# dvnam1605/MAACO-path-planing

Hardware: NVIDIA B200
Metric: path evals/sec (MAACO ant tours, MPA/PSO/GA fitness) at 1/2/4/8 B200 vs CPU (higher is better)
Workload: dtype f64

## Files before the change

### maaco_path_planing_b200/csrc/mpp_maaco.cu

```cuda
#include <type_traits>
#include <cmath>
#include <cstdlib>
#include <thread>
#include <vector>

#include "mpp_common.cuh"

static inline double hdist(int r0, int c0, int r1, int c1) {
    long long dr = r0 - r1, dc = c0 - c1;
    return std::sqrt((double)(dr * dr + dc * dc));
}

extern "C" double mpp_maaco_q0(int K, int k, double q0_initial) {
    double k0 = 0.7 * (double)K, q0;
    if ((double)k < k0) {
        if (std::fabs((double)K - k0) < 1e-6) q0 = q0_initial;
        else q0 = ((double)(K - k) / (double)K) * q0_initial;
    } else {
        double q0_at_k0 = (((double)K - k0) / (double)K) * q0_initial;
        q0 = q0_at_k0 +
             (((double)k - k0) / ((double)K - k0 + 1e-9)) * (q0_initial * (1 - ((double)K - k0) / (double)K) / 2.0);
    }
    q0 = q0 > 0.01 ? q0 : 0.01;
    return q0 < 0.99 ? q0 : 0.99;
// ... 466 lines not shown
        const uint32_t need0 = __ballot_sync(0xffffffffu, active && ((unsigned)lrow - edge_lo > edge_span || (unsigned)lcol - edge_lo > edge_span));
        if (!__any_sync(0xffffffffu, active)) break;
        if ((step & gmask) == 0 || need0) {
            if ((step & gmask) == 0) {
                const int la = lane & (apw - 1);
                const mpp_u4 rb = mpp_philox(step + (uint32_t)(lane / apw), (uint32_t)(A.ant_offset + a0 + la), A.it,
                                             MPP_CLS_MAACO_TOUR, key0, key1);
                const double u0 = mpp_u53(rb.x, rb.y), u1 = mpp_u53(rb.z, rb.w);
                const bool greedy = u0 <= A.q0;
                uint32_t pack = greedy ? (1u << 24) : 0u;
#pragma unroll
                for (int n = 2; n <= 8; ++n) {
                    int k = (int)(u1 * (double)n);
                    k = k < n ? k : n - 1;
                    pack |= (uint32_t)k << (3 * (n - 1));
                }
                const uint32_t k2 = (pack >> 3) & 7u, k3 = (pack >> 6) & 7u;
                uint32_t pack2 = (greedy ? (1u << 16) : 0u) | (0u << 2) | (1u << 4) | (2u << 8);
                pack2 |= (k2 ? 1u : 0u) << 6;
                pack2 |= (k2 ? 2u : 0u) << 10;
                pack2 |= (k2 ? 2u : 1u) << 12;
                pack2 |= k3 << 14;
                __syncwarp();
                rngu[lane] = make_double2(u0, u1);
                rngp[lane] = pack;
                rngq[lane] = pack2;
                __syncwarp();
            }
            uint32_t need = need0;
            while (need) {
                const int src = __ffs(need) - 1;
                const int s_lrow = __shfl_sync(0xffffffffu, lrow, src), s_lcol = __shfl_sync(0xffffffffu, lcol, src);
                const int s_wr = __shfl_sync(0xffffffffu, wr, src), s_wc = __shfl_sync(0xffffffffu, wc, src);
                const int a_s = a0 + src;
                uint2 *const w_s = win_w + src * 64;
                int d_wr = 0, d_wc = 0;
                if ((unsigned)s_lrow - edge_lo > edge_span) {
                    const bool up = s_lrow < U;
                    d_wr = up ? -1 : 1;
                    const int t_out = up ? s_wr + 1 : s_wr, t_in = up ? s_wr - 1 : s_wr + 2;
                    const uint2 keep = w_s[up ? lane : lane + 32], out = w_s[up ? lane + 32 : lane];
                    tour_tile_store(V, a_s, t_out, s_wc, lane, out.x);
                    tour_tile_store(V, a_s, t_out, s_wc + 1, lane, out.y);
                    uint2 nw;
                    nw.x = tour_tile_load(V, a_s, t_in, s_wc, lane);
                    nw.y = tour_tile_load(V, a_s, t_in, s_wc + 1, lane);
                    w_s[up ? lane + 32 : lane] = keep;
                    w_s[up ? lane : lane + 32] = nw;
                } else {
                    const bool left = s_lcol < U;
                    d_wc = left ? -1 : 1;
                    const int t_out = left ? s_wc + 1 : s_wc, t_in = left ? s_wc - 1 : s_wc + 2;
                    const uint2 o0 = w_s[lane], o1 = w_s[lane + 32];
                    tour_tile_store(V, a_s, s_wr, t_out, lane, left ? o0.y : o0.x);
                    tour_tile_store(V, a_s, s_wr + 1, t_out, lane, left ? o1.y : o1.x);
                    const uint32_t x0 = tour_tile_load(V, a_s, s_wr, t_in, lane);
                    const uint32_t x1 = tour_tile_load(V, a_s, s_wr + 1, t_in, lane);
                    w_s[lane] = left ? make_uint2(x0, o0.x) : make_uint2(o0.y, x0);
                    w_s[lane + 32] = left ? make_uint2(x1, o1.x) : make_uint2(o1.y, x1);
                }
#ifdef MPP_TOUR_STATS
                if (lane == src) ++st_slides;
#endif
                if (lane == src) {
                    wr += d_wr; wc += d_wc;
                    lrow -= d_wr << 5; lcol -= d_wc << 5;
                    prow_s -= (uint32_t)(d_wr * 256);
                }
                __syncwarp();
                const bool again = (lane == src) && ((unsigned)lrow - edge_lo > edge_span || (unsigned)lcol - edge_lo > edge_span);
                need = (need & (need - 1)) | __ballot_sync(0xffffffffu, again);
            }
        }
        uint32_t slot = (step & gmask) * slot_bytes;
        for (int su = 0; su < U; ++su, slot += slot_bytes)
        if (active) {
            int m = -1, dcur = 0, dpr = 0, dcc = 0, dphi = 0;
            double dl = 0.0;
            if (!(fw2 & 1u)) {
                const uint32_t p2 = lds_u32(rngq_s + slot);
                const uint32_t A3 = (fw2 >> 1) & 7u;
                uint32_t pool;
#ifdef MPP_TOUR_STATS
                if (gap == 0) ++st_t1; else ++st_t2;
#endif
                if (gap == 0) {
                    pool = (p2 & 0x10000u) ? ((fw2 >> 25) & 7u) : A3;
                } else {
                    const uint2 ra = lds_u2(prow_s + k_dpr0), rb = lds_u2(prow_s + k_dpr1), rc = lds_u2(prow_s + k_dpr2);
                    const int c0 = lcol + k_dc0, c1 = lcol + k_dc1, c2 = lcol + k_dc2;
                    const uint32_t v0 = ((c0 & 32) ? ra.y : ra.x) >> (c0 & 31);
                    const uint32_t v1 = ((c1 & 32) ? rb.y : rb.x) >> (c1 & 31);
                    const uint32_t v2 = ((c2 & 32) ? rc.y : rc.x) >> (c2 & 31);
                    const uint32_t c3 = A3 & ~((v0 & 1u) | ((v1 & 1u) << 1) | ((v2 & 1u) << 2));
                    pool = (p2 & 0x10000u) ? ((fw2 >> (1u + 3u * c3)) & 7u) : c3;
                    if (c3 == 0u) pool = 0u;
                }
                if (pool != 0u) {
                    const uint32_t mem = (p2 >> (2u * pool)) & 3u;
                    const uint4 fv = lds_u4(sbase_k + T1_FAST_OFF + 16u * mem);
                    dl = lds_f64(sbase_k + T1_FLEN_OFF + 8u * mem);
                    dcur = (int)fv.x; dpr = (int)fv.y; dcc = (int)fv.z;
                    m = (int)(fv.w & 0xFFu);
                    dphi = (int)(fv.w >> 8);
                    const uint32_t m1 = 0u - (mem & 1u), m2 = 0u - (mem >> 1);
                    uint32_t t;
                    asm("lop3.b32 %0, %1, %2, %3, 0xD8;" : "=r"(t) : "r"(bq.x), "r"(bq.y), "r"(m1));
                    asm("lop3.b32 %0, %1, %2, %3, 0xD8;" : "=r"(fw2) : "r"(t), "r"(bq.z), "r"(m2));
                }
            }
#ifdef MPP_TOUR_STATS
            if (m < 0) { ++st_t3; if (!(fw2 & 1u)) { if (gap == 0) --st_t1; else --st_t2; } }
#endif
            if (m < 0) {
                const uint32_t ctx = (n_path >= 2) ? (uint32_t)(prev_m + 1) : 0u;
                const uint32_t fw = ldg32_nc_pinned(rank_fast + (size_t)cur * 9 + ctx);
                const uint2 rws = ldg64_pinned(rank_slow + (size_t)cur * 9 + ctx);
                uint2 nb = make_uint2(0u, 0u);
                if (fast_ok) nb = ldg64_pinned(nb8 + cur);
                const uint32_t pack = lds_u32(rngp_s + slot);
                const uint2 q0r = lds_u2(prow_s - 8u), q1r = lds_u2(prow_s), q2r = lds_u2(prow_s + 8u);
                const int rot = lcol - 1;
                const bool sw = rot & 32;
                const uint32_t t3 = __funnelshift_r(sw ? q0r.y : q0r.x, q0r.y, rot) & 7u;
                const uint32_t m3 = __funnelshift_r(sw ? q1r.y : q1r.x, q1r.y, rot) & 5u;
                const uint32_t b3 = __funnelshift_r(sw ? q2r.y : q2r.x, q2r.y, rot) & 7u;
                const uint32_t vis = t3 | ((m3 & 1u) << 3) | ((m3 & 4u) << 2) | (b3 << 5);
                const uint32_t valid = (fw >> 24) & ~vis;
                uint32_t cand = valid & P1;
                if (cand == 0u) {
                    cand = valid & orient_mask(tr - cur / C, tc - cur % C);
                    if (!cand) cand = valid;
                }
                if (cand == 0u) {
                    failed = true;
                    active = false;
                } else {
                    if ((cand & (cand - 1u)) == 0u) {
                        m = __ffs(cand) - 1;
                    } else if ((fw & 7u) != 0u) {
                        const double2 uu = rngu[(slot >> 2) + lane];
                        m = tour_select_slow(cand, cur / C, cur % C, C, n_path >= 2, prev_m, tau_m, E01_m, A.alpha, A.q0, uu.x, uu.y);
                    } else {
                        uint32_t pool = cand;
                        if (pack & (1u << 24)) {
                            const uint2 sp = lds_u2(sbase_k + T1_SPREAD_OFF + 8u * cand);
                            const uint32_t f0 = __byte_perm(sp.x, sp.y, rws.x & 0xFFFFu), f1 = __byte_perm(sp.x, sp.y, rws.x >> 16);
                            const uint32_t ff = f0 ? f0 : f1;
                            const int pos4 = ((__ffs(ff) - 1) >> 1) + (f0 ? 0 : 16);
                            const uint32_t best = (rws.x >> pos4) & 7u;
                            pool = cand & ~((1u << best) - 1u);
                        }
                        const int n = __popc(pool);
                        const int k = (pack >> (3 * n - 3)) & 7u;
                        m = (int)lds_u8(sbase_k + T1_KTH_OFF + pool * 8u + (uint32_t)k);
                    }
                    const uint4 mvv = lds_u4(sbase_k + T1_MOVE_OFF + 16u * (uint32_t)m);
                    dcur = (int)mvv.x; dpr = (int)mvv.y; dcc = (int)mvv.z; dphi = (int)mvv.w;
                    dl = lds_f64(sbase_k + T1_DLEN_OFF + 8u * (uint32_t)m);
                    if (fast_ok) {
                        const uint32_t by = (((m & 4) ? nb.y : nb.x) >> (8 * (m & 3))) & 0xFFu;
                        const uint32_t fl = lds_u32(sbase_k + T1_FLD_OFF + 4u * (by >> 4));
                        const uint32_t A3n = (by >> 1) & 7u;
                        const uint32_t Gn = A3n ? ((fl >> (3u * (A3n - 1u))) & 7u) : 0u;
                        fw2 = (by & 1u) | (A3n << 1) | (fl << 4) | (Gn << 25);
                    }
                }
            }
            if (active) {
                cur += dcur;
                if (fast_ok) bq = ldg128_pinned(bundle + cur);
                gap -= dphi;
                gap = gap > 0 ? gap : 0;
                prow_s += (uint32_t)dpr;
                lrow += dpr >> 3;
                lcol += dcc;
                asm volatile("red.shared.or.b32 [%0], %1;" ::"r"(prow_s + 4u * ((uint32_t)lcol >> 5)), "r"(1u << (lcol & 31)) : "memory");
                if (n_path <= k_max_cells) *mvp = (uint8_t)m;
                ++mvp;
                len += dl;
                if (m != prev_m) ++turns;
                prev_m = m;
                ++n_path;
                if (cur == k_target || n_path >= k_max_path) active = false;
#ifdef MPP_TOUR_STATS
                st_c1 = clock64();
#endif
            }
        }
    }
    for (int src = 0; src < apw && a0 + src < A.n_ants; ++src) {
        const int s_wr = __shfl_sync(0xffffffffu, wr, src), s_wc = __shfl_sync(0xffffffffu, wc, src);
        const uint2 o0 = win_w[src * 64 + lane], o1 = win_w[src * 64 + lane + 32];
        tour_tile_store(V, a0 + src, s_wr, s_wc, lane, o0.x);
        tour_tile_store(V, a0 + src, s_wr, s_wc + 1, lane, o0.y);
        tour_tile_store(V, a0 + src, s_wr + 1, s_wc, lane, o1.x);
        tour_tile_store(V, a0 + src, s_wr + 1, s_wc + 1, lane, o1.y);
    }
    if (lane < apw && a < A.n_ants) {
        const bool ok = !failed && cur == target;
        mpp_ant_result res;
        res.length = ok ? len : __longlong_as_double(0x7ff0000000000000ll);
        res.n_cells = ok ? n_path : 0;
        res.turns = ok ? (turns > 0 ? turns : 0) : -1;
        A.result[(size_t)map * A.result_stride + A.ant_offset + a] = res;
        if constexpr (P2P)
            for (int g = 0; g < PA.n_peers; ++g) PA.peer_result[g][A.ant_offset + a] = res;
        if (A.steps) atomicAdd(A.steps, (unsigned long long)(n_path - 1));
#ifdef MPP_TOUR_STATS
        int *st = (int *)(A.moves + ((size_t)map * A.n_ants + a + 1) * A.max_cells - 32);
        st[0] = st_t1; st[1] = st_t2; st[2] = st_t3; st[3] = st_slides; st[4] = (int)(st_c1 - st_c0); st[5] = n_path - 1;
        st[6] = ok ? 1 : 0;
#endif
    }
}

static int colony_check(const mpp_map_batch *maps, const mpp_colony *c, const char *who) {
    MPP_REQUIRE(maps && c, "%s: null argument", who);
    MPP_REQUIRE(c->tau && c->E01 && c->rank && c->slabs && c->touched && c->moves && c->result && c->deposit && c->okbits &&
                    c->state && c->best_cells && c->seeds, "%s: null colony buffer", who);
    MPP_REQUIRE(c->max_cells > 0 && c->tau_stride >= (long long)maps->rows * maps->cols, "%s: bad max_cells / tau_stride", who);
    for (int k = 0; k < maps->n_maps; ++k)
        MPP_REQUIRE(maps->meta_host[k].start >= 0 && maps->meta_host[k].target >= 0, "%s: map %d has no start/target", who, k);
    return MPP_OK;
}

static int tours_launch(const mpp_map_batch *maps, const mpp_colony *c, int iteration, double q0, double alpha,
                        int n_ants, int ant_offset, int n_ants_total, int ants_per_warp,
                        uint32_t *const *peer_slabs, uint32_t *const *peer_touched, mpp_ant_result *const *peer_result,
                        int n_peers, int rows_per_rank, void *stream) {
    int rc = colony_check(maps, c, "mpp_maaco_tours");
    if (rc) return rc;
    MPP_REQUIRE(n_ants > 0 && ant_offset >= 0 && ant_offset + n_ants <= n_ants_total, "mpp_maaco_tours: bad ant range");
    MPP_CUDA(cudaSetDevice(maps->device));
    const RankLayout L = rank_layout(maps->rows, maps->cols);
    const int TR = tiles_r(maps->rows);
    TourArgs A;
    A.meta = maps->meta_dev;
    A.rank = c->rank; A.rank_stride = L.total_words; A.rank_margin = L.margin; A.rank_fast_words = L.fast_words;
    A.rank_bundle_words = L.bundle_words; A.rank_nb8_words = L.nb8_words;
    A.R = maps->rows; A.C = maps->cols;
    A.tau = c->tau; A.tau_stride = (size_t)c->tau_stride; A.E01 = c->E01; A.E01_stride = (size_t)c->E01_stride;
    A.it = (uint32_t)iteration; A.q0 = q0; A.alpha = alpha;
    A.n_ants = n_ants; A.ant_offset = ant_offset;
    A.seeds = c->seeds;
    const size_t tw = (size_t)mpp_maaco_touched_words(TR, maps->cols, n_ants) / 2;
    A.slabs = c->slabs; A.slab_stride = (size_t)mpp_maaco_slab_words(TR, maps->cols, n_ants);
    A.touched = c->touched + (size_t)(iteration & 1) * tw * maps->n_maps; A.touched_stride = tw;
    A.moves = c->moves; A.max_cells = c->max_cells;
    A.result = c->result; A.result_stride = (size_t)n_ants_total;
    A.steps = c->steps; A.latch = c->latch;
    TourPeers PA;
    for (int g = 0; g < MPP_MAX_PEERS; ++g) {
        PA.peer_slabs[g] = g < n_peers ? peer_slabs[g] : nullptr;
        PA.peer_touched[g] = g < n_peers ? peer_touched[g] : nullptr;
        PA.peer_result[g] = g < n_peers ? peer_result[g] : nullptr;
    }
    PA.n_peers = n_peers; PA.rows_per_rank = rows_per_rank; PA.n_total = n_ants_total;
    int apw = 16;
    const char *e = getenv("MPP_TOUR_APW");
    if (e) apw = atoi(e);
    else if (ants_per_warp) apw = ants_per_warp;
    else {
        const long long total = (long long)n_ants * maps->n_maps;
        while (apw > 2 && (total + apw - 1) / apw < 12ll * maps->sm_count) apw >>= 1;
    }
    MPP_REQUIRE(apw == 1 || apw == 2 || apw == 4 || apw == 8 || apw == 16 || apw == 32,
                "ants per warp (MPP_TOUR_APW / ants_per_warp) must be a power of two <= 32");
    const int warps = (n_ants + apw - 1) / apw, wpb = MPP_TOUR1_THREADS / 32;
    const size_t smem = T1_WIN_OFF + (size_t)wpb * apw * 512;
    {
        static size_t smem_set[64] = {0};
        const int dv = maps->device & 63;
        if (smem > smem_set[dv]) {
            MPP_CUDA(cudaFuncSetAttribute(mpp_maaco_tour1_kernel<false>, cudaFuncAttributeMaxDynamicSharedMemorySize, (int)smem));
            MPP_CUDA(cudaFuncSetAttribute(mpp_maaco_tour1_kernel<true>, cudaFuncAttributeMaxDynamicSharedMemorySize, (int)smem));
            smem_set[dv] = smem;
        }
    }
    const dim3 grid((warps + wpb - 1) / wpb, maps->n_maps);
    if (n_peers > 0) mpp_maaco_tour1_kernel<true><<<grid, MPP_TOUR1_THREADS, smem, (cudaStream_t)stream>>>(A, apw, PA);
    else mpp_maaco_tour1_kernel<false><<<grid, MPP_TOUR1_THREADS, smem, (cudaStream_t)stream>>>(A, apw, TourNoPeers());
    MPP_CUDA(cudaGetLastError());
    return MPP_OK;
}

extern "C" int mpp_maaco_tours(const mpp_map_batch *maps, const mpp_colony *c, int iteration, double q0, double alpha,
                               int n_ants, int ant_offset, int n_ants_total, int ants_per_warp, void *stream) {
    return tours_launch(maps, c, iteration, q0, alpha, n_ants, ant_offset, n_ants_total, ants_per_warp, nullptr, nullptr,
                        nullptr, 0, 1, stream);
}

extern "C" int mpp_maaco_tours_p2p(const mpp_map_batch *maps, const mpp_colony *c, int iteration, double q0, double alpha,
                                   int n_ants, int ant_offset, int n_ants_total, int ants_per_warp,
                                   uint32_t *const *slabs_peers, uint32_t *const *touched_peers,
                                   mpp_ant_result *const *result_peers, int n_peers, int tile_rows_per_rank, void *stream) {
    MPP_REQUIRE(maps && maps->n_maps == 1, "mpp_maaco_tours_p2p: a sharded colony is one map");
    MPP_REQUIRE(slabs_peers && touched_peers && result_peers && n_peers > 0 && n_peers <= MPP_MAX_PEERS && tile_rows_per_rank > 0 &&
                    (long long)n_peers * tile_rows_per_rank >= tiles_r(maps->rows), "mpp_maaco_tours_p2p: bad peer arguments");
    return tours_launch(maps, c, iteration, q0, alpha, n_ants, ant_offset, n_ants_total, ants_per_warp, slabs_peers,
                        touched_peers, result_peers, n_peers, tile_rows_per_rank, stream);
}

__global__ void __launch_bounds__(128) mpp_maaco_rank_kernel(const uint8_t *__restrict__ svalid_all,
                                                             const double *__restrict__ tau_all, size_t tau_stride,
                                                             const double *__restrict__ E01_all, size_t E01_stride,
                                                             double alpha, int R, int C,
                                                             const MppMapMeta *__restrict__ meta, uint32_t *__restrict__ rank_all,
                                                             size_t rank_stride, size_t rank_margin, size_t rank_fast_words,
                                                             size_t rank_bundle_words, size_t rank_nb8_words,
                                                             const int32_t *__restrict__ latch) {
    const int cell = blockIdx.x * 128 + threadIdx.x;
    if (cell >= R * C) return;
    if (latch && *latch) return;
    const int map = blockIdx.y;
    const uint8_t *svalid = svalid_all + (size_t)map * R * C;
    const double *tau = tau_all + (size_t)map * tau_stride;
    const double *E01 = E01_all + (size_t)map * E01_stride;
    uint32_t *rank_fast = rank_all + (size_t)map * rank_stride + rank_margin;
    uint2 *rank_slow = (uint2 *)(rank_all + (size_t)map * rank_stride + rank_fast_words);
    uint32_t *bundle = rank_all + (size_t)map * rank_stride + rank_bundle_words;
    uint8_t *nb8 = (uint8_t *)(rank_all + (size_t)map * rank_stride + rank_nb8_words);
    const uint32_t P1 = meta[map].s1.P1;
    const uint32_t sv = svalid[cell];
    double a0[8], a1[8];
#pragma unroll
    for (int m = 0; m < 8; ++m) {
        a0[m] = a1[m] = -1.0;
        if ((sv >> m) & 1u) {
            const int j = cell + ((int)((0xA940u >> (2 * m)) & 3u) - 1) * C + ((int)((0x9224u >> (2 * m)) & 3u) - 1);
            const double tv = tau[j];
            const double ta = (alpha == 1.0) ? tv : pow_slow(tv, alpha);
            const double2 e = *(const double2 *)(E01 + 2 * (size_t)j);
            a0[m] = ta * e.x;
            a1[m] = ta * e.y;
        }
    }
    const bool p1_three = __popc(P1) == 3;
    const int s0 = __ffs(P1) - 1, s1 = __ffs(P1 & (P1 - 1)) - 1, s2 = 31 - __clz(P1);
    for (int ctx = 0; ctx < 9; ++ctx) {
        double a[8];
#pragma unroll
        for (int m = 0; m < 8; ++m) a[m] = (ctx > 0 && m != ctx - 1) ? a1[m] : a0[m];
        double cmx = 0.0;
#pragma unroll
        for (int m = 0; m < 8; ++m) cmx = fmax(cmx, a[m]);
        uint32_t word = 0xFFFFFFu, perm = 0u, fast = 7u, order = 0u;
        if (cmx < 1e-10) {
            word = 0u;
#pragma unroll
            for (int m = 0; m < 8; ++m) {
                int pos = 0;
#pragma unroll
                for (int q = 0; q < 8; ++q) pos += (a[q] > a[m]) || (a[q] == a[m] && q < m);
                word |= (uint32_t)pos << (3 * m);
                perm |= (uint32_t)m << (4 * pos);
            }
            fast = 0u;
            if (p1_three) {
                const uint32_t p0 = (word >> (3 * s0)) & 7u, p1 = (word >> (3 * s1)) & 7u, p2 = (word >> (3 * s2)) & 7u;
                order = (p0 < p1 ? 1u : 0u) | (p0 < p2 ? 2u : 0u) | (p1 < p2 ? 4u : 0u);
#pragma unroll
                for (uint32_t c = 1; c < 8; ++c) {
                    uint32_t bp = 8u, bi = 0u;
                    if ((c & 1u) && p0 < bp) { bp = p0; bi = 0u; }
                    if ((c & 2u) && p1 < bp) { bp = p1; bi = 1u; }
                    if ((c & 4u) && p2 < bp) { bp = p2; bi = 2u; }
                    fast |= (c & ~((1u << bi) - 1u)) << (3u * c);
                }
            }
        }
        const size_t t = (size_t)cell * 9 + ctx;
        rank_fast[t] = fast | (sv << 24);
        rank_slow[t] = make_uint2(perm, word | (sv << 24));
        if (p1_three && ctx > 0) {
            const int mv = ctx - 1;
            const int pr = cell / C - ((int)((0xA940u >> (2 * mv)) & 3u) - 1), pc = cell % C - ((int)((0x9224u >> (2 * mv)) & 3u) - 1);
            if (pr >= 0 && pr < R && pc >= 0 && pc < C) {
                const uint32_t A3 = ((sv >> s0) & 1u) | (((sv >> s1) & 1u) << 1) | (((sv >> s2) & 1u) << 2);
                nb8[((size_t)pr * C + pc) * 8 + mv] = (uint8_t)((fast & 7u ? 1u : 0u) | (A3 << 1) | (order << 4));
                const int k = (ctx == s0 + 1) ? 0 : ((ctx == s1 + 1) ? 1 : ((ctx == s2 + 1) ? 2 : -1));
                if (k >= 0) bundle[((size_t)pr * C + pc) * 4 + k] = tour_word2(fast | (sv << 24), s0, s1, s2);
            }
        }
    }
}

extern "C" int mpp_maaco_rank(const mpp_map_batch *maps, const mpp_colony *c, double alpha, void *stream) {
    int rc = colony_check(maps, c, "mpp_maaco_rank");
    if (rc) return rc;
    MPP_CUDA(cudaSetDevice(maps->device));
    const int total = maps->rows * maps->cols;
    const RankLayout L = rank_layout(maps->rows, maps->cols);
    mpp_maaco_rank_kernel<<<dim3((total + 127) / 128, maps->n_maps), 128, 0, (cudaStream_t)stream>>>(
        maps->svalid_dev, c->tau, (size_t)c->tau_stride, c->E01, (size_t)c->E01_stride, alpha, maps->rows, maps->cols,
        maps->meta_dev, c->rank, L.total_words, L.margin, L.fast_words, L.bundle_words, L.nb8_words, c->latch);
    MPP_CUDA(cudaGetLastError());
    return MPP_OK;
}

#define MPP_BEST_THREADS 1024
__device__ __forceinline__ bool lt_len_idx(double la, int ia, double lb, int ib) {
    return la < lb || (la == lb && ia < ib);
}
__device__ __forceinline__ int move_delta(uint32_t m, int C) {
    return ((int)((0xA940u >> (2 * m)) & 3u) - 1) * C + ((int)((0x9224u >> (2 * m)) & 3u) - 1);
}

__global__ void __launch_bounds__(MPP_BEST_THREADS)
mpp_maaco_best_kernel(const mpp_ant_result *__restrict__ res_all, const uint8_t *__restrict__ moves_all, int max_cells,
                      int moves_ant_offset, int moves_n_ants, int n, double Q, int iteration, int C,
                      const MppMapMeta *__restrict__ meta, mpp_maaco_state *state_all, int32_t *best_cells_all,
                      double *deposit_all, uint32_t *okbits_all, double *log_all, int log_rows,
                      const int32_t *__restrict__ latch) {
    __shared__ double s_len[32];
    __shared__ int s_idx[32];
    __shared__ int s_t[32];
    __shared__ double b_len;
    __shared__ int b_r, b_ant, b_turns, b_copy, s_base;
    if (latch && *latch) return;
    const int map = blockIdx.x;
    const mpp_ant_result *res = res_all + (size_t)map * n;
    double *deposit = deposit_all + (size_t)map * n;
    uint32_t *okbits = okbits_all + (size_t)map * ((n + 31) >> 5);
    mpp_maaco_state *state = state_all + map;
    const int tid = threadIdx.x, lane = tid & 31, wid = tid >> 5;
    const double INF = __longlong_as_double(0x7ff0000000000000ll);
    double ml = INF;
    int mi = 0x7fffffff;
    for (int i0 = 0; i0 < n; i0 += MPP_BEST_THREADS) {
        const int i = i0 + tid;
        bool dep = false;
        if (i < n) {
            const mpp_ant_result ri = res[i];
            const double l = ri.length;
            if (lt_len_idx(l, i, ml, mi)) { ml = l; mi = i; }
            dep = (l != INF && ri.n_cells > 0 && l > 1e-6);
            deposit[i] = dep ? Q / l : 0.0;
        }
        const uint32_t ok = __ballot_sync(0xffffffffu, dep);
        if (lane == 0 && i < n) okbits[i >> 5] = ok;
    }
#pragma unroll
    for (int o = 16; o; o >>= 1) {
        const double ol = __shfl_xor_sync(0xffffffffu, ml, o);
        const int oi = __shfl_xor_sync(0xffffffffu, mi, o);
        if (lt_len_idx(ol, oi, ml, mi)) { ml = ol; mi = oi; }
    }
    if (lane == 0) { s_len[wid] = ml; s_idx[wid] = mi; }
    __syncthreads();
    if (wid == 0) {
        ml = s_len[lane]; mi = s_idx[lane];
#pragma unroll
        for (int o = 16; o; o >>= 1) {
            const double ol = __shfl_xor_sync(0xffffffffu, ml, o);
            const int oi = __shfl_xor_sync(0xffffffffu, mi, o);
            if (lt_len_idx(ol, oi, ml, mi)) { ml = ol; mi = oi; }
        }
        if (lane == 0) { b_len = ml; b_r = mi; }
    }
    __syncthreads();
    const double L = b_len;
    const int r = b_r;
    int bt = 0x7fffffff, bi = 0x7fffffff;
    if (L != INF) {
        for (int i = tid; i < n; i += MPP_BEST_THREADS) {
            if (i < r) continue;
            const mpp_ant_result ri = res[i];
            const double l = ri.length;
            if (i == r || fabs(l - L) < 1e-9) {
                const int t = ri.turns;
                if (t >= 0 && (t < bt || (t == bt && i < bi))) { bt = t; bi = i; }
            }
        }
    }
#pragma unroll
    for (int o = 16; o; o >>= 1) {
        const int ot = __shfl_xor_sync(0xffffffffu, bt, o), oi = __shfl_xor_sync(0xffffffffu, bi, o);
        if (ot < bt || (ot == bt && oi < bi)) { bt = ot; bi = oi; }
    }
    if (lane == 0) { s_t[wid] = bt; s_idx[wid] = bi; }
    __syncthreads();
    if (wid == 0) {
        bt = s_t[lane]; bi = s_idx[lane];
#pragma unroll
        for (int o = 16; o; o >>= 1) {
            const int ot = __shfl_xor_sync(0xffffffffu, bt, o), oi = __shfl_xor_sync(0xffffffffu, bi, o);
            if (ot < bt || (ot == bt && oi < bi)) { bt = ot; bi = oi; }
        }
        if (lane == 0) {
            const bool any = (L != INF);
            b_ant = any ? bi : -1;
            b_turns = any ? bt : -1;
            mpp_maaco_state st = *state;
            int copy = 0;
            if (any) {
                if (L < st.best_len) {
                    st.best_len = L; st.best_turns = bt; copy = 1;
                } else if (fabs(L - st.best_len) < 1e-9) {
                    if (bt < st.best_turns) { st.best_turns = bt; copy = 1; }
                }
            }
            if (copy) { st.best_n_cells = res[bi].n_cells; st.best_iter = iteration; st.best_ant = bi; }
            st.iter_best_len = L; st.iter_best_turns = b_turns; st.iter_best_ant = b_ant;
            *state = st;
            b_copy = copy;
            if (log_all && iteration >= 1 && iteration <= log_rows) {
                double *lg = log_all + ((size_t)map * log_rows + (size_t)(iteration - 1)) * 4;
                lg[0] = L; lg[1] = (double)b_turns; lg[2] = st.best_len; lg[3] = (double)st.best_turns;
            }
        }
    }
    __syncthreads();
    if (b_copy && b_ant >= moves_ant_offset && b_ant < moves_ant_offset + moves_n_ants) {
        const int a = b_ant - moves_ant_offset;
        int nm = res[b_ant].n_cells - 1;
        if (nm > max_cells) nm = max_cells;
        const uint8_t *mv = moves_all + ((size_t)map * moves_n_ants + a) * max_cells;
        int32_t *out = best_cells_all + (size_t)map * (max_cells + 1);
        if (tid == 0) { out[0] = meta[map].start; s_base = meta[map].start; }
        __syncthreads();
        for (int k0 = 0; k0 < nm; k0 += MPP_BEST_THREADS) {
            const int k = k0 + tid;
            int x = (k < nm) ? move_delta(mv[k], C) : 0;
#pragma unroll
            for (int o = 1; o < 32; o <<= 1) { const int y = __shfl_up_sync(0xffffffffu, x, o); if (lane >= o) x += y; }
            if (lane == 31) s_idx[wid] = x;
            __syncthreads();
            if (wid == 0) {
                int w = s_idx[lane];
#pragma unroll
                for (int o = 1; o < 32; o <<= 1) { const int y = __shfl_up_sync(0xffffffffu, w, o); if (lane >= o) w += y; }
                s_idx[lane] = w;
            }
            __syncthreads();
            const int cell = s_base + (wid ? s_idx[wid - 1] : 0) + x;
            if (k < nm) out[k + 1] = cell;
            __syncthreads();
            if (tid == MPP_BEST_THREADS - 1) s_base = cell;
            __syncthreads();
        }
    }
}

extern "C" int mpp_maaco_best(const mpp_map_batch *maps, const mpp_colony *c, int moves_ant_offset, int moves_n_ants,
                              int n_ants_total, double Q, int iteration, void *stream) {
    int rc = colony_check(maps, c, "mpp_maaco_best");
    if (rc) return rc;
    MPP_REQUIRE(n_ants_total > 0 && iteration >= 1, "mpp_maaco_best: n_ants=%d iteration=%d", n_ants_total, iteration);
    MPP_CUDA(cudaSetDevice(maps->device));
    mpp_maaco_best_kernel<<<maps->n_maps, MPP_BEST_THREADS, 0, (cudaStream_t)stream>>>(
        c->result, c->moves, c->max_cells, moves_ant_offset, moves_n_ants, n_ants_total, Q, iteration, maps->cols,
        maps->meta_dev, c->state, c->best_cells, c->deposit, c->okbits, c->log, c->log_rows, c->latch);
    MPP_CUDA(cudaGetLastError());
    return MPP_OK;
}

#define MPP_PHER_THREADS 256
#define MPP_PHER_CHUNK 2048
#define PHER_TRIP 128
#define PHER_PITCH 132

__device__ __forceinline__ double pher_finalize(double t, int r, int c, const uint32_t *occ, int pitch, int R, int C,
                                                double rho, const mpp_maaco_state *state) {
    double b = state->best_len;
    if (b == __longlong_as_double(0x7ff0000000000000ll)) b = (double)(R + C);
    if (b < 1e-6) b = 1e-6;
    const double tmax = (1.0 / (1.0 - rho)) * (1.0 / b);
    int mx = C > R ? C : R;
    if (mx < 1) mx = 1;
    const double tmin = tmax / (2.0 * (double)mx);
    const int pb = c + 1;
    const bool obst = (occ[(r + 1) * pitch + (pb >> 5)] >> (pb & 31)) & 1u;
    if (obst) return 1e-9;
    t = t > tmin ? t : tmin;
    return t < tmax ? t : tmax;
}

struct PherArgs {
    const uint32_t *occ; int occ_words, pitch, R, C;
    double *tau; size_t tau_stride;
    uint32_t *slabs; size_t slab_stride;
    uint32_t *touched, *touched_next;
    size_t touched_stride;
    const double *deposit; const uint32_t *okbits;
    int n_ants;
    int tile_row0;
    double rho;
    const mpp_maaco_state *state;
    int clear_slabs;
    const int32_t *latch;
    double *const *tau_peers; int n_peers;
    const MppMapMeta *meta;
};

#ifdef MPP_PHER_PROF
__device__ unsigned long long g_pher_prof[8192 * 8];
extern "C" int mpp_debug_pher_prof(unsigned long long *out) {
    return cudaMemcpyFromSymbol(out, g_pher_prof, sizeof(g_pher_prof)) == cudaSuccess ? 0 : -1;
}
__device__ __forceinline__ unsigned long long gtimer() { unsigned long long t; asm volatile("mov.u64 %0, %globaltimer;" : "=l"(t)); return t; }
#endif

#ifndef MPP_PHER_MINB
#define MPP_PHER_MINB 7
#endif
__global__ void __launch_bounds__(MPP_PHER_THREADS, MPP_PHER_MINB) mpp_maaco_pheromone_kernel(const PherArgs A) {
    __shared__ int s_list[MPP_PHER_CHUNK];
#ifdef MPP_PHER_PROF
    const unsigned long long prof_t0 = gtimer();
    unsigned long long prof_hits = 0, prof_rounds = 0, prof_list = 0, prof_loop = 0, prof_tl = 0;
#endif
    __shared__ uint32_t s_w[2][8][PHER_PITCH];
    __shared__ __align__(16) double s_d[2][PHER_TRIP];
    __shared__ int s_wcnt[2];
    if (A.latch && *A.latch) return;
#ifdef MPP_PHER_ONLY
    if ((blockIdx.x >> 2) != MPP_PHER_ONLY) return;
#endif
    const int lane = threadIdx.x & 31, wid = threadIdx.x >> 5, map = blockIdx.y;
    const int TC = (A.C + 31) >> 5;
    int tile_l = blockIdx.x >> 2;
    const int rg = blockIdx.x & 3;
    {
        const int nt = gridDim.x >> 2;
        const MppMapMeta &MM = A.meta[map];
        int h0 = ((MM.start / A.C >> 5) - A.tile_row0) * TC + (MM.start % A.C >> 5);
        int h1 = ((MM.target / A.C >> 5) - A.tile_row0) * TC + (MM.target % A.C >> 5);
        if (h0 < 0 || h0 >= nt) h0 = -1;
        if (h1 < 0 || h1 >= nt || h1 == h0) h1 = -1;
        if (h0 < 0) { h0 = h1; h1 = -1; }
        const int nh = (h0 >= 0) + (h1 >= 0);
        if (tile_l < nh) {
            tile_l = tile_l == 0 ? h0 : h1;
        } else {
            const int lo = (nh == 2 && h1 < h0) ? h1 : h0, hi = (nh == 2 && h1 < h0) ? h0 : h1;
            tile_l -= nh;
            if (nh >= 1 && tile_l >= lo) ++tile_l;
            if (nh == 2 && tile_l >= hi) ++tile_l;
        }
    }
    const int trow = A.tile_row0 + tile_l / TC, tcx = tile_l % TC;
    const int row_in_tile = rg * 8 + wid;
    const int r = (trow << 5) + row_in_tile, c = (tcx << 5) + lane;
    const bool live = r < A.R && c < A.C;
    double *tau = A.tau + (size_t)map * A.tau_stride;
    const int NW = (A.n_ants + 31) >> 5;
    const uint32_t *tb = A.touched + (size_t)map * A.touched_stride + (size_t)tile_l * NW;
    const uint32_t *ok = A.okbits + (size_t)map * NW;
    uint32_t *slab_t = A.slabs + (size_t)map * A.slab_stride + (size_t)tile_l * A.n_ants * 32 + row_in_tile;
    const double *dep = A.deposit + (size_t)map * A.n_ants;
    double t = 0.0;
    if (live) t = tau[(size_t)r * A.C + c] * (1.0 - A.rho);
    for (int w0 = 0; w0 < NW; w0 += MPP_PHER_CHUNK / 32) {
#ifdef MPP_PHER_PROF
        prof_tl = gtimer();
#endif
        int cnt = 0;
        uint32_t bits = 0u;
        if (wid < 2) {
            const int w = w0 + wid * 32 + lane;
            if (w < NW) bits = tb[w] & ok[w];
            cnt = __popc(bits);
            int x = cnt;
#pragma unroll
            for (int o = 1; o < 32; o <<= 1) { const int y = __shfl_up_sync(0xffffffffu, x, o); if (lane >= o) x += y; }
            if (lane == 31) s_wcnt[wid] = x;
            cnt = x - cnt;
        }
        __syncthreads();
        const int k = s_wcnt[0] + s_wcnt[1];
        if (wid < 2) {
            int o = cnt + (wid ? s_wcnt[0] : 0);
            const int abase = (w0 + wid * 32 + lane) << 5;
            while (bits) { const int b = __ffs(bits) - 1; bits &= bits - 1; s_list[o++] = abase + b; }
        }
        __syncthreads();
#ifdef MPP_PHER_PROF
        { const unsigned long long g_ = gtimer(); prof_list += g_ - prof_tl; prof_tl = g_; }
#endif
        const int ntrip = (k + PHER_TRIP - 1) / PHER_TRIP;
        const uint32_t *slab_g = slab_t - wid + (threadIdx.x & 1) * 4;
        uint4 wv = make_uint4(0u, 0u, 0u, 0u);
        double dv = 0.0;
        int av = -1;
        auto issue = [&](int trip) {
            const int i = trip * PHER_TRIP + (threadIdx.x >> 1);
            wv = make_uint4(0u, 0u, 0u, 0u); av = -1; dv = 0.0;
            if (i < k) { av = s_list[i]; wv = *(const uint4 *)(slab_g + (size_t)av * 32); }
            if (threadIdx.x < PHER_TRIP) {
                const int i2 = trip * PHER_TRIP + threadIdx.x;
                if (i2 < k) dv = dep[s_list[i2]];
            }
        };
        issue(0);
        for (int trip = 0; trip < ntrip; ++trip) {
            const int buf = trip & 1;
// ... 331 lines not shown
```

Measured before the change: 5.993 million.

## Tile rank kernel in 2D with shared-memory staging and pull-based neighbor bytes

Restructures the MAACO rank kernel into 32x8 cell tiles. It computes all nine context rank words at once from pairwise comparison masks instead of a per-context O(64) rank loop, and stages the fast and slow rank outputs in shared memory so they are written back coalesced. Neighbor nb8 and bundle entries are now pulled by each cell from a shared halo rather than scattered to neighbors, with halo cells recomputed redundantly. This trades extra halo compute and shared memory for fewer divergent scattered global writes and less comparison work.

After: 6.137 million (median of 6 runs). 1.02x the previous value.

```diff
diff --git a/maaco_path_planing_b200/csrc/mpp_maaco.cu b/maaco_path_planing_b200/csrc/mpp_maaco.cu
--- a/maaco_path_planing_b200/csrc/mpp_maaco.cu
+++ b/maaco_path_planing_b200/csrc/mpp_maaco.cu
@@ -792,86 +792,179 @@
                         touched_peers, result_peers, n_peers, tile_rows_per_rank, stream);
 }
 
-__global__ void __launch_bounds__(128) mpp_maaco_rank_kernel(const uint8_t *__restrict__ svalid_all,
-                                                             const double *__restrict__ tau_all, size_t tau_stride,
-                                                             const double *__restrict__ E01_all, size_t E01_stride,
-                                                             double alpha, int R, int C,
-                                                             const MppMapMeta *__restrict__ meta, uint32_t *__restrict__ rank_all,
-                                                             size_t rank_stride, size_t rank_margin, size_t rank_fast_words,
-                                                             size_t rank_bundle_words, size_t rank_nb8_words,
-                                                             const int32_t *__restrict__ latch) {
-    const int cell = blockIdx.x * 128 + threadIdx.x;
-    if (cell >= R * C) return;
+#define RANK_TW 32
+#define RANK_TH 8
+#define RANK_THREADS (RANK_TW * RANK_TH)
+#define RANK_HW (RANK_TW + 2)
+#define RANK_NHALO (2 * RANK_HW + 2 * RANK_TH)
+
+__device__ __forceinline__ void rank_values(int r, int c, int C, uint32_t sv, const double *__restrict__ tau,
+                                            const double *__restrict__ E01, double alpha, double a0[8], double a1[8]) {
+    double tv[8];
+    double2 e[8];
+#pragma unroll
+    for (int m = 0; m < 8; ++m) {
+        const int j = ((sv >> m) & 1u) ? (r + (int)((0xA940u >> (2 * m)) & 3u) - 1) * C + c + (int)((0x9224u >> (2 * m)) & 3u) - 1
+                                       : r * C + c;
+        tv[m] = tau[j];
+        e[m] = *(const double2 *)(E01 + 2 * (size_t)j);
+    }
+#pragma unroll
+    for (int m = 0; m < 8; ++m) {
+        a0[m] = a1[m] = -1.0;
+        if ((sv >> m) & 1u) {
+            const double ta = (alpha == 1.0) ? tv[m] : pow_slow(tv[m], alpha);
+            a0[m] = ta * e[m].x;
+            a1[m] = ta * e[m].y;
+        }
+    }
+}
+
+__device__ __forceinline__ void rank_words(const double a0[8], const double a1[8], uint32_t w[9], uint32_t &small) {
+    uint32_t S0[8], S1[8], X[8];
+#pragma unroll
+    for (int p = 0; p < 8; ++p) S0[p] = S1[p] = X[p] = 0u;
+#pragma unroll
+    for (int q = 0; q < 8; ++q)
+#pragma unroll
+        for (int m = q + 1; m < 8; ++m) {
+            if (a0[q] >= a0[m]) S0[q] |= 1u << (3 * m); else S0[m] |= 1u << (3 * q);
+            if (a1[q] >= a1[m]) S1[q] |= 1u << (3 * m); else S1[m] |= 1u << (3 * q);
+            if (a0[q] >= a1[m]) X[q] |= 1u << (3 * m);
+            if (a0[m] > a1[q]) X[m] |= 1u << (3 * q);
+        }
+    uint32_t W0 = 0u, W1 = 0u, n0 = 0u, n1 = 0u;
+#pragma unroll
+    for (int p = 0; p < 8; ++p) {
+        W0 += S0[p];
+        W1 += S1[p];
+        n0 |= (a0[p] >= 1e-10 ? 1u : 0u) << p;
+        n1 |= (a1[p] >= 1e-10 ? 1u : 0u) << p;
+    }
+    w[0] = W0;
+    small = n0 ? 0u : 1u;
+#pragma unroll
+    for (int p = 0; p < 8; ++p) {
+        w[p + 1] = ((W1 - S1[p] + X[p]) & ~(7u << (3 * p))) | ((7u - (uint32_t)__popc(X[p])) << (3 * p));
+        small |= (((n0 >> p) & 1u) == 0u && (n1 & ~(1u << p)) == 0u ? 1u : 0u) << (p + 1);
+    }
+}
+__device__ __forceinline__ uint32_t rank_order(uint32_t word, int s0, int s1, int s2) {
+    const uint32_t p0 = (word >> (3 * s0)) & 7u, p1 = (word >> (3 * s1)) & 7u, p2 = (word >> (3 * s2)) & 7u;
+    return (p0 < p1 ? 1u : 0u) | (p0 < p2 ? 2u : 0u) | (p1 < p2 ? 4u : 0u);
+}
+
+__global__ void __launch_bounds__(RANK_THREADS, 3) mpp_maaco_rank_kernel(const uint8_t *__restrict__ svalid_all,
+                                                                      const double *__restrict__ tau_all, size_t tau_stride,
+                                                                      const double *__restrict__ E01_all, size_t E01_stride,
+                                                                      double alpha, int R, int C,
+                                                                      const MppMapMeta *__restrict__ meta, uint32_t *__restrict__ rank_all,
+                                                                      size_t rank_stride, size_t rank_margin, size_t rank_fast_words,
+                                                                      size_t rank_bundle_words, size_t rank_nb8_words,
+                                                                      const int32_t *__restrict__ latch) {
+    __shared__ uint32_t s_fields[8];
+    __shared__ uint2 s_nbp[(RANK_TH + 2) * RANK_HW];
+    __shared__ uint32_t s_fast[RANK_TH][RANK_TW * 9];
+    __shared__ uint2 s_slow[RANK_TH][RANK_TW * 9];
     if (latch && *latch) return;
     const int map = blockIdx.y;
+    const int tcols = (C + RANK_TW - 1) / RANK_TW;
+    const int r0 = (blockIdx.x / tcols) * RANK_TH, c0 = (blockIdx.x % tcols) * RANK_TW;
+    const int tx = threadIdx.x % RANK_TW, ty = threadIdx.x / RANK_TW;
     const uint8_t *svalid = svalid_all + (size_t)map * R * C;
     const double *tau = tau_all + (size_t)map * tau_stride;
     const double *E01 = E01_all + (size_t)map * E01_stride;
-    uint32_t *rank_fast = rank_all + (size_t)map * rank_stride + rank_margin;
-    uint2 *rank_slow = (uint2 *)(rank_all + (size_t)map * rank_stride + rank_fast_words);
-    uint32_t *bundle = rank_all + (size_t)map * rank_stride + rank_bundle_words;
-    uint8_t *nb8 = (uint8_t *)(rank_all + (size_t)map * rank_stride + rank_nb8_words);
     const uint32_t P1 = meta[map].s1.P1;
-    const uint32_t sv = svalid[cell];
-    double a0[8], a1[8];
-#pragma unroll
-    for (int m = 0; m < 8; ++m) {
-        a0[m] = a1[m] = -1.0;
-        if ((sv >> m) & 1u) {
-            const int j = cell + ((int)((0xA940u >> (2 * m)) & 3u) - 1) * C + ((int)((0x9224u >> (2 * m)) & 3u) - 1);
-            const double tv = tau[j];
-            const double ta = (alpha == 1.0) ? tv : pow_slow(tv, alpha);
-            const double2 e = *(const double2 *)(E01 + 2 * (size_t)j);
-            a0[m] = ta * e.x;
-            a1[m] = ta * e.y;
-        }
-    }
     const bool p1_three = __popc(P1) == 3;
     const int s0 = __ffs(P1) - 1, s1 = __ffs(P1 & (P1 - 1)) - 1, s2 = 31 - __clz(P1);
-    for (int ctx = 0; ctx < 9; ++ctx) {
-        double a[8];
-#pragma unroll
-        for (int m = 0; m < 8; ++m) a[m] = (ctx > 0 && m != ctx - 1) ? a1[m] : a0[m];
-        double cmx = 0.0;
-#pragma unroll
-        for (int m = 0; m < 8; ++m) cmx = fmax(cmx, a[m]);
-        uint32_t word = 0xFFFFFFu, perm = 0u, fast = 7u, order = 0u;
-        if (cmx < 1e-10) {
-            word = 0u;
-#pragma unroll
-            for (int m = 0; m < 8; ++m) {
-                int pos = 0;
-#pragma unroll
-                for (int q = 0; q < 8; ++q) pos += (a[q] > a[m]) || (a[q] == a[m] && q < m);
-                word |= (uint32_t)pos << (3 * m);
-                perm |= (uint32_t)m << (4 * pos);
-            }
-            fast = 0u;
-            if (p1_three) {
-                const uint32_t p0 = (word >> (3 * s0)) & 7u, p1 = (word >> (3 * s1)) & 7u, p2 = (word >> (3 * s2)) & 7u;
-                order = (p0 < p1 ? 1u : 0u) | (p0 < p2 ? 2u : 0u) | (p1 < p2 ? 4u : 0u);
-#pragma unroll
-                for (uint32_t c = 1; c < 8; ++c) {
-                    uint32_t bp = 8u, bi = 0u;
-                    if ((c & 1u) && p0 < bp) { bp = p0; bi = 0u; }
-                    if ((c & 2u) && p1 < bp) { bp = p1; bi = 1u; }
-                    if ((c & 4u) && p2 < bp) { bp = p2; bi = 2u; }
-                    fast |= (c & ~((1u << bi) - 1u)) << (3u * c);
+    if (threadIdx.x < 8) s_fields[threadIdx.x] = tour_fields(threadIdx.x);
+    __syncthreads();
+    const int r = r0 + ty, c = c0 + tx;
+    const bool inside = r < R && c < C;
+    uint32_t sv = 0u, A3 = 0u;
+    uint2 nbp = make_uint2(0u, 0u);
+    if (inside) {
+        sv = svalid[(size_t)r * C + c];
+        A3 = ((sv >> s0) & 1u) | (((sv >> s1) & 1u) << 1) | (((sv >> s2) & 1u) << 2);
+        double a0[8], a1[8];
+        rank_values(r, c, C, sv, tau, E01, alpha, a0, a1);
+        uint32_t w[9], small;
+        rank_words(a0, a1, w, small);
+#pragma unroll
+        for (int ctx = 0; ctx < 9; ++ctx) {
+            uint32_t word = 0xFFFFFFu, perm = 0u, fast = 7u, b = 1u | (A3 << 1);
+            if ((small >> ctx) & 1u) {
+                word = w[ctx];
+#pragma unroll
+                for (int m = 0; m < 8; ++m) perm |= (uint32_t)m << (4 * ((word >> (3 * m)) & 7u));
+                fast = 0u;
+                if (p1_three) {
+                    const uint32_t order = rank_order(word, s0, s1, s2);
+                    fast = s_fields[order] << 3;
+                    b = (A3 << 1) | (order << 4);
                 }
             }
-        }
-        const size_t t = (size_t)cell * 9 + ctx;
-        rank_fast[t] = fast | (sv << 24);
-        rank_slow[t] = make_uint2(perm, word | (sv << 24));
-        if (p1_three && ctx > 0) {
-            const int mv = ctx - 1;
-            const int pr = cell / C - ((int)((0xA940u >> (2 * mv)) & 3u) - 1), pc = cell % C - ((int)((0x9224u >> (2 * mv)) & 3u) - 1);
-            if (pr >= 0 && pr < R && pc >= 0 && pc < C) {
-                const uint32_t A3 = ((sv >> s0) & 1u) | (((sv >> s1) & 1u) << 1) | (((sv >> s2) & 1u) << 2);
-                nb8[((size_t)pr * C + pc) * 8 + mv] = (uint8_t)((fast & 7u ? 1u : 0u) | (A3 << 1) | (order << 4));
-                const int k = (ctx == s0 + 1) ? 0 : ((ctx == s1 + 1) ? 1 : ((ctx == s2 + 1) ? 2 : -1));
-                if (k >= 0) bundle[((size_t)pr * C + pc) * 4 + k] = tour_word2(fast | (sv << 24), s0, s1, s2);
+            s_fast[ty][tx * 9 + ctx] = fast | (sv << 24);
+            s_slow[ty][tx * 9 + ctx] = make_uint2(perm, word | (sv << 24));
+            if (ctx >= 1 && ctx <= 4) nbp.x |= b << (8 * (ctx - 1));
+            if (ctx >= 5) nbp.y |= b << (8 * (ctx - 5));
+        }
+    }
+    s_nbp[(ty + 1) * RANK_HW + tx + 1] = nbp;
+    if (p1_three && threadIdx.x < RANK_NHALO) {
+        const int h = threadIdx.x;
+        int hr, hc;
+        if (h < 2 * RANK_HW) { hr = (h < RANK_HW) ? 0 : RANK_TH + 1; hc = h % RANK_HW; }
+        else { hr = 1 + (h - 2 * RANK_HW) / 2; hc = ((h - 2 * RANK_HW) & 1) ? RANK_HW - 1 : 0; }
+        const int rr = r0 + hr - 1, cc = c0 + hc - 1;
+        uint2 nbp = make_uint2(0u, 0u);
+        if (rr >= 0 && rr < R && cc >= 0 && cc < C) {
+            const uint32_t svh = svalid[(size_t)rr * C + cc];
+            const uint32_t A3h = ((svh >> s0) & 1u) | (((svh >> s1) & 1u) << 1) | (((svh >> s2) & 1u) << 2);
+            double a0[8], a1[8];
+            rank_values(rr, cc, C, svh, tau, E01, alpha, a0, a1);
+            uint32_t w[9], small;
+            rank_words(a0, a1, w, small);
+#pragma unroll
+            for (int ctx = 1; ctx < 9; ++ctx) {
+                const uint32_t b = ((small >> ctx) & 1u) ? ((A3h << 1) | (rank_order(w[ctx], s0, s1, s2) << 4)) : (1u | (A3h << 1));
+                if (ctx <= 4) nbp.x |= b << (8 * (ctx - 1));
+                else nbp.y |= b << (8 * (ctx - 5));
             }
+        }
+        s_nbp[hr * RANK_HW + hc] = nbp;
+    }
+    __syncthreads();
+    uint32_t *rank = rank_all + (size_t)map * rank_stride;
+    if (inside && p1_three) {
+        const uint8_t *nbb = (const uint8_t *)s_nbp;
+        uint32_t lo = 0u, hi = 0u;
+#pragma unroll
+        for (int mv = 0; mv < 8; ++mv) {
+            const int hr = ty + (int)((0xA940u >> (2 * mv)) & 3u), hc = tx + (int)((0x9224u >> (2 * mv)) & 3u);
+            const uint32_t b = nbb[(hr * RANK_HW + hc) * 8 + mv];
+            if (mv < 4) lo |= b << (8 * mv); else hi |= b << (8 * (mv - 4));
+        }
+        const size_t cell = (size_t)r * C + c;
+        ((uint2 *)(rank + rank_nb8_words))[cell] = make_uint2(lo, hi);
+        uint32_t w2[3];
+#pragma unroll
+        for (int k = 0; k < 3; ++k) {
+            const int sk = k == 0 ? s0 : (k == 1 ? s1 : s2);
+            const uint32_t b = (((sk < 4) ? lo : hi) >> (8 * (sk & 3))) & 0xFFu;
+            const uint32_t An = (b >> 1) & 7u, F = s_fields[b >> 4];
+            w2[k] = (b & 1u) ? (1u | (An << 1)) : ((An << 1) | (F << 4) | ((An ? (F >> (3u * (An - 1u))) & 7u : 0u) << 25));
+        }
+        ((uint4 *)(rank + rank_bundle_words))[cell] = make_uint4(w2[0], w2[1], w2[2], 0u);
+    }
+    const int nv = min(RANK_TW, C - c0);
+    if (r < R) {
+        const size_t base = ((size_t)r * C + c0) * 9;
+        uint32_t *fast_out = rank + rank_margin + base;
+        uint2 *slow_out = (uint2 *)(rank + rank_fast_words) + base;
+        for (int i = tx; i < 9 * nv; i += RANK_TW) {
+            fast_out[i] = s_fast[ty][i];
+            slow_out[i] = s_slow[ty][i];
         }
     }
 }
@@ -880,9 +973,9 @@
     int rc = colony_check(maps, c, "mpp_maaco_rank");
     if (rc) return rc;
     MPP_CUDA(cudaSetDevice(maps->device));
-    const int total = maps->rows * maps->cols;
+    const int tiles = ((maps->rows + RANK_TH - 1) / RANK_TH) * ((maps->cols + RANK_TW - 1) / RANK_TW);
     const RankLayout L = rank_layout(maps->rows, maps->cols);
-    mpp_maaco_rank_kernel<<<dim3((total + 127) / 128, maps->n_maps), 128, 0, (cudaStream_t)stream>>>(
+    mpp_maaco_rank_kernel<<<dim3(tiles, maps->n_maps), RANK_THREADS, 0, (cudaStream_t)stream>>>(
         maps->svalid_dev, c->tau, (size_t)c->tau_stride, c->E01, (size_t)c->E01_stride, alpha, maps->rows, maps->cols,
         maps->meta_dev, c->rank, L.total_words, L.margin, L.fast_words, L.bundle_words, L.nb8_words, c->latch);
     MPP_CUDA(cudaGetLastError());
```
